# microsoft/ptgnn

Measured on AMD Instinct MI355X. Metric: edges/sec per MP layer, higher is better.
Workload: dtype f32; 1 GPU; cfg3: Graph2Class-style batch, 48 graphs N=115772, T0=8->T=17, E=625130 (incl. reverse+self), Typilus GGNN arch: 8 GGNN layers H=128 (+concat residual), max; hidden=128, mode=forward (inference), fp32, plan_build_in_step=True, message_rows=shared per (edge type, source) pair, parallelism=single GPU, minibatches_rotated=4

## Files before the change

ptgnn_amd/csrc/stream_gemm.hip:

```cpp
#include <stdlib.h>

#include "dense_common.h"
#include <atomic>

#include "stream_gemm.h"

namespace ptgnn_amd {
namespace {

using u32x4 = __attribute__((ext_vector_type(4))) uint32_t;

constexpr int kLdsBudget = 160 * 1024;
constexpr size_t kEpiBytes = 16 + 8 * 8 * 36 * sizeof(float);

__device__ __forceinline__ f32x16 zero16() {
  f32x16 v;
#pragma unroll
  for (int r = 0; r < 16; ++r) v[r] = 0.f;
  return v;
}

struct ARows {
  const float *c0, *c1, *n0, *n1;
};

__device__ __forceinline__ float4 load_piece(const ARows &r, int cc, int ch0, int nch, int g) {
  const bool nx = cc >= nch;
  const int c = nx ? cc - nch : cc;
  const float *b0 = nx ? r.n0 : r.c0;
  const float *b1 = nx ? r.n1 : r.c1;
  const float *p = c < ch0 ? b0 + c * 32 : b1 + (c - ch0) * 32;
  return *reinterpret_cast<const float4 *>(p + g * 8);
}

__device__ __forceinline__ int lane_piece_offset(int hi) { return hi * 4; }

template <int NBLK, int NACC, int PH, bool GRU>
__device__ __forceinline__ void chunk_f32(f32x16 (&acc)[NACC], float4 (&buf)[4], float4 (&bcur)[NBLK],
                                          const float *bl, int cbs, int kofs, int kofs_next, const ARows &rows,
                                          int cnext, int ch0, int nch) {
#pragma unroll
  for (int g = 0; g < 4; ++g) {
    float4 bn[NBLK];
    const int ko = g < 3 ? kofs + (g + 1) * 8 : kofs_next;
#pragma unroll
    for (int n = 0; n < NBLK; ++n) bn[n] = *reinterpret_cast<const float4 *>(bl + n * cbs + ko);
    __builtin_amdgcn_sched_barrier(0);
    const float4 a = buf[g];
#define PTGNN_STEP(C)                                                                     \
    _Pragma("unroll") for (int n = 0; n < NBLK; ++n) {                                    \
      const int t = (GRU && PH == 1 && n == 2) ? 3 : n;                                   \
      acc[t] = __builtin_amdgcn_mfma_f32_32x32x2f32(a.C, bcur[n].C, acc[t], 0, 0, 0);     \
    }
    PTGNN_STEP(x) PTGNN_STEP(y) PTGNN_STEP(z) PTGNN_STEP(w)
#undef PTGNN_STEP
    __builtin_amdgcn_sched_barrier(0);
#pragma unroll
    for (int n = 0; n < NBLK; ++n) bcur[n] = bn[n];
  }
#pragma unroll
  for (int g = 0; g < 4; ++g) {
    buf[g] = load_piece(rows, cnext, ch0, nch, g);
    __builtin_amdgcn_sched_barrier(0);
  }
}

struct Slab {
  int ld;
  __device__ __forceinline__ Slab(int K, int ) { ld = K + 4; }
  static size_t bytes(int K, int rows) { return (size_t)rows * (K + 4) * 4; }

  __device__ __forceinline__ void put4(float *smem, int r, int k, float4 v) const {
    *reinterpret_cast<float4 *>(smem + r * ld + k) = v;
  }
};

template <int NT, typename SrcFn, typename LiveFn>
__device__ __forceinline__ void fill_slab(float *smem, const Slab &sl, int rows, int kq, SrcFn src, LiveFn live) {
  constexpr int UB = 8;
  const int total = rows * kq;
  for (int i0 = threadIdx.x; i0 < total; i0 += NT * UB) {
    float4 v[UB];
    int rr[UB], qq[UB];
#pragma unroll
    for (int u = 0; u < UB; ++u) {
      const int i = i0 + u * NT;
      const int ic = i < total ? i : total - 1;
      rr[u] = ic / kq;
      qq[u] = ic - rr[u] * kq;
    }
#pragma unroll
    for (int u = 0; u < UB; ++u) {
      v[u] = *reinterpret_cast<const float4 *>(src(rr[u], qq[u]));
      __builtin_amdgcn_sched_barrier(0);
    }
#pragma unroll
    for (int u = 0; u < UB; ++u) {
      if (i0 + u * NT < total) sl.put4(smem, rr[u], qq[u] * 4, live(rr[u]) ? v[u] : make_float4(0.f, 0.f, 0.f, 0.f));
    }
  }
}

template <int NBLK, int NACC, bool GRU>
__device__ __forceinline__ void unit_kloop(f32x16 (&acc)[NACC], float4 (&a0)[4], float4 (&a1)[4],
                                           const float *smem, const Slab &sl, int li, int hi,
                                           const ARows &rows, int ch0, int nch) {
  const float *bl = smem + li * sl.ld + hi * 4;
  const int cbs = 32 * sl.ld;
  const int e0 = GRU ? ch0 : nch;
  float4 bcur[NBLK];
#pragma unroll
  for (int n = 0; n < NBLK; ++n) bcur[n] = *reinterpret_cast<const float4 *>(bl + n * cbs);
  for (int c = 0; c < e0; c += 2) {
    const int kn = c + 2 < nch ? c * 32 + 64 : 0;
    chunk_f32<NBLK, NACC, 0, GRU>(acc, a0, bcur, bl, cbs, c * 32, c * 32 + 32, rows, c + 2, ch0, nch);
    chunk_f32<NBLK, NACC, 0, GRU>(acc, a1, bcur, bl, cbs, c * 32 + 32, kn, rows, c + 3, ch0, nch);
  }
  if constexpr (GRU) {
    for (int c = ch0; c < nch; c += 2) {
      const int kn = c + 2 < nch ? c * 32 + 64 : 0;
      chunk_f32<NBLK, NACC, 1, GRU>(acc, a0, bcur, bl, cbs, c * 32, c * 32 + 32, rows, c + 2, ch0, nch);
      chunk_f32<NBLK, NACC, 1, GRU>(acc, a1, bcur, bl, cbs, c * 32 + 32, kn, rows, c + 3, ch0, nch);
    }
  }
}

__device__ __forceinline__ void prologue_loads(float4 (&a0)[4], float4 (&a1)[4], const ARows &rows, int ch0,
                                               int nch) {
#pragma unroll
  for (int g = 0; g < 4; ++g) {
    a0[g] = load_piece(rows, 0, ch0, nch, g);
    __builtin_amdgcn_sched_barrier(0);
  }
#pragma unroll
  for (int g = 0; g < 4; ++g) {
    a1[g] = load_piece(rows, 1, ch0, nch, g);
    __builtin_amdgcn_sched_barrier(0);
  }
}

__device__ __forceinline__ void unit_fence() {
  __builtin_amdgcn_s_waitcnt(0x0F70);
  __builtin_amdgcn_sched_barrier(0);
}

__device__ __forceinline__ int claim_unit(int *counter) {
  int v = 0;
  if ((threadIdx.x & 63) == 0) v = atomicAdd(counter, 1);
  return __builtin_amdgcn_readfirstlane(v);
}

constexpr int kTqLd = 36;
constexpr int kTqFloats = 8 * kTqLd;

__device__ __forceinline__ float4 tq_transpose(float *tq, int lane, int li, int hi, float v0, float v1, float v2,
                                               float v3) {
  float *w = tq + (4 * hi) * kTqLd + li;
  w[0] = v0; w[kTqLd] = v1; w[2 * kTqLd] = v2; w[3 * kTqLd] = v3;
  __builtin_amdgcn_wave_barrier();
  const float4 o = *reinterpret_cast<const float4 *>(tq + (lane >> 3) * kTqLd + (lane & 7) * 4);
  __builtin_amdgcn_wave_barrier();
  return o;
}

__device__ __forceinline__ void tq_untranspose(float *tq, int lane, int li, int hi, float4 in, float (&v)[4]) {
  *reinterpret_cast<float4 *>(tq + (lane >> 3) * kTqLd + (lane & 7) * 4) = in;
  __builtin_amdgcn_wave_barrier();
  const float *r = tq + (4 * hi) * kTqLd + li;
  v[0] = r[0]; v[1] = r[kTqLd]; v[2] = r[2 * kTqLd]; v[3] = r[3 * kTqLd];
  __builtin_amdgcn_wave_barrier();
}

using u32x4 = __attribute__((ext_vector_type(4))) uint32_t;

__device__ __forceinline__ __amdgpu_buffer_rsrc_t rows_descriptor(float *base , int64_t ld, int64_t rows_left,
                                                                  int width ) {
  const uint64_t b = reinterpret_cast<uint64_t>(base);
  const uint32_t lo = __builtin_amdgcn_readfirstlane((uint32_t)b), hi = __builtin_amdgcn_readfirstlane((uint32_t)(b >> 32));
  const int64_t rows = rows_left < 32 ? rows_left : 32;
  const int64_t bytes = rows > 0 ? ((rows - 1) * ld + width) * 4 : 0;
  return __builtin_amdgcn_make_buffer_rsrc(reinterpret_cast<float *>(((uint64_t)hi << 32) | lo), 0,
                                           __builtin_amdgcn_readfirstlane((int)bytes), 0x00020000);
}

__device__ __forceinline__ void store_row4(__amdgpu_buffer_rsrc_t rsrc, int lane_bytes, int uniform_bytes, float4 o) {
  const u32x4 v = {__float_as_uint(o.x), __float_as_uint(o.y), __float_as_uint(o.z), __float_as_uint(o.w)};
  __builtin_amdgcn_raw_buffer_store_b128(v, rsrc, lane_bytes + uniform_bytes, 0, 0);
}

template <int ACT, bool BIAS = true>
__device__ __forceinline__ void store_block_tq(const f32x16 &c, float *tq, float *yblk ,
                                               int64_t ld_y, float bv, int64_t rows_left, int lane, int li, int hi,
                                               const float *addblk = nullptr, int64_t ld_add = 0) {
  auto val = [&](int r) { return BIAS ? act_apply<ACT>(c[r] + bv) : act_apply<ACT>(c[r]); };
  float4 addv[4];
  if (addblk) {
#pragma unroll
    for (int q = 0; q < 4; ++q) {
      int64_t r = 8 * q + (lane >> 3);
      r = r < rows_left ? r : rows_left - 1;
      addv[q] = *reinterpret_cast<const float4 *>(addblk + r * ld_add + (lane & 7) * 4);
    }
  }
// ... 46 lines not shown

template <int NB>
__device__ __forceinline__ void linear_epilogue(const LinearArgs &p, f32x16 (&acc)[NB], float *tq, int64_t row0,
                                                int col_base, int lane, int li, int hi) {
#pragma unroll
  for (int n = 0; n < NB; ++n) {
    const int col = col_base + n * 32 + li;
    if (col_base + n * 32 < p.n_out) {
      const float bv = p.bias ? p.bias[col] : 0.f;
      if (p.vec_store) {
        float *yb = p.y + row0 * p.ld_y + col_base + n * 32;
        const int64_t left = p.rows - row0;
        if (p.bias) {
#pragma unroll
          for (int r = 0; r < 16; ++r) acc[n][r] += bv;
        }
        const float *ab = p.addend ? p.addend + row0 * p.ld_add + col_base + n * 32 : nullptr;
        if (p.act == PTGNN_AMD_ACT_TANH) store_block_tq<PTGNN_AMD_ACT_TANH, false>(acc[n], tq, yb, p.ld_y, 0.f, left, lane, li, hi, ab, p.ld_add);
        else if (p.act == PTGNN_AMD_ACT_RELU) store_block_tq<PTGNN_AMD_ACT_RELU, false>(acc[n], tq, yb, p.ld_y, 0.f, left, lane, li, hi, ab, p.ld_add);
        else store_block_tq<PTGNN_AMD_ACT_NONE, false>(acc[n], tq, yb, p.ld_y, 0.f, left, lane, li, hi, ab, p.ld_add);
      } else {
        float *yp = p.y + (row0 + 4 * hi) * p.ld_y + col;
        if (p.act == PTGNN_AMD_ACT_TANH) store_block<PTGNN_AMD_ACT_TANH>(acc[n], yp, p.ld_y, bv, row0, p.rows, hi);
        else if (p.act == PTGNN_AMD_ACT_RELU) store_block<PTGNN_AMD_ACT_RELU>(acc[n], yp, p.ld_y, bv, row0, p.rows, hi);
        else store_block<PTGNN_AMD_ACT_NONE>(acc[n], yp, p.ld_y, bv, row0, p.rows, hi);
      }
    }
    acc[n] = zero16();
  }
}

template <int NB>
__global__ __launch_bounds__(512, 2) void k_stream_linear(LinearArgs p) {
  extern __shared__ __attribute__((aligned(16))) float smem[];
  constexpr int NT = 512, BN = 32 * NB;
  const int b = blockIdx.x, G = gridDim.x;
  int slab, part;
  if (G % (kNumXcd * p.ncs) == 0) {
    const int xcd = b % kNumXcd, j = b / kNumXcd;
    slab = j % p.ncs;
    part = xcd + kNumXcd * (j / p.ncs);
  } else {
    slab = b / p.rps;
    part = b % p.rps;
  }
  const int rb0 = part * p.run_len;
  const int rb1 = rb0 + p.run_len < p.nrb ? rb0 + p.run_len : p.nrb;
  if (rb0 >= rb1) return;
  const int count = rb1 - rb0;

  const Slab sl(p.K, BN);
  int *counter = reinterpret_cast<int *>(smem + p.lds_floats);
  float *const tq = smem + p.lds_floats + 4 + (threadIdx.x >> 6) * kTqFloats;
  if (threadIdx.x == 0) *counter = 0;
  const int col_base = slab * BN;
  fill_slab<NT>(smem, sl, BN, p.K >> 2,
                       [&](int r, int q) {
                         const int wr = col_base + r < p.n_out ? col_base + r : p.n_out - 1;
                         return p.w + (int64_t)wr * p.K + q * 4;
                       },
                       [&](int r) { return col_base + r < p.n_out; });
  __syncthreads();

  const int lane = threadIdx.x & 63;
  const int li = lane & 31, hi = lane >> 5;
  const int nch = p.K >> 5;
  const int lofs = lane_piece_offset(hi);
  auto rowp = [&](int u) {
    int64_t row = (int64_t)(rb0 + (u < count ? u : count - 1)) * 32 + li;
    row = row < p.rows ? row : p.rows - 1;
    return p.x + row * p.ld_x + lofs;
  };
  int cur = claim_unit(counter);
  if (cur >= count) return;
  int nxt = claim_unit(counter);
  ARows rows;
  rows.c0 = rows.c1 = rowp(cur);
  rows.n0 = rows.n1 = rowp(nxt);
  float4 a0[4], a1[4];
  prologue_loads(a0, a1, rows, nch, nch);
  f32x16 acc[NB];
#pragma unroll
  for (int n = 0; n < NB; ++n) acc[n] = zero16();

  while (cur < count) {
    const int nn = claim_unit(counter);
    unit_fence();
    unit_kloop<NB, NB, false>(acc, a0, a1, smem, sl, li, hi, rows, nch, nch);
    const int64_t row0 = (int64_t)(rb0 + cur) * 32;
    linear_epilogue<NB>(p, acc, tq, row0, col_base, lane, li, hi);
    cur = nxt;
    nxt = nn;
    rows.c0 = rows.c1 = rows.n0;
    rows.n0 = rows.n1 = rowp(nxt);
  }
}

struct GruArgs {
  const float *a; int64_t ld_a; const float *h; int64_t ld_h;
  const float *w_ih, *w_hh, *b_ih, *b_hh;
  int64_t n; int M, H;
  float *out; int64_t ld_out; float *gates;
  int nrb, ncs, rps, run_len;
  int lds_floats;
};

__device__ __forceinline__ float fast_sigmoid(float v) {
  return __builtin_amdgcn_rcpf(1.0f + __builtin_amdgcn_exp2f(-1.4426950408889634f * v));
}

using f32x2 = __attribute__((ext_vector_type(2))) float;
__device__ __forceinline__ f32x2 splat2(float v) { return f32x2{v, v}; }
__device__ __forceinline__ f32x2 rcp_1_plus_exp2(f32x2 t) {
  const f32x2 d = f32x2{__builtin_amdgcn_exp2f(t.x), __builtin_amdgcn_exp2f(t.y)} + splat2(1.0f);
  return f32x2{__builtin_amdgcn_rcpf(d.x), __builtin_amdgcn_rcpf(d.y)};
}

__device__ __forceinline__ void gru_epilogue(const GruArgs &p, const f32x16 (&acc)[4], float *tq, int64_t row0,
                                             int j0, int lane, int li, int hi, float bir, float biz, float bin,
                                             float bhr, float bhz, float bhn) {
  const int trow = lane >> 3, tcol = (lane & 7) * 4;
#ifndef PTGNN_GLOBAL_STORES
  const __amdgpu_buffer_rsrc_t out_rsrc = rows_descriptor(p.out + row0 * p.ld_out + j0, p.ld_out, p.n - row0, 32);
  const __amdgpu_buffer_rsrc_t gate_rsrc =
      rows_descriptor(p.gates ? p.gates + row0 * (int64_t)(4 * p.H) + j0 : p.out, 4 * (int64_t)p.H, p.n - row0, 3 * p.H + 32);
#endif
#pragma unroll
  for (int q = 0; q < 4; ++q) {
    int64_t hrow = row0 + 8 * q + trow;
    const bool rvalid = hrow < p.n;
    hrow = rvalid ? hrow : p.n - 1;
    float hp[4];
    tq_untranspose(tq, lane, li, hi, *reinterpret_cast<const float4 *>(p.h + hrow * p.ld_h + j0 + tcol), hp);
// ... 18 lines not shown
    }
    const float4 o = tq_transpose(tq, lane, li, hi, res[0], res[1], res[2], res[3]);
#ifdef PTGNN_GLOBAL_STORES
    if (rvalid) *reinterpret_cast<float4 *>(p.out + hrow * p.ld_out + j0 + tcol) = o;
#else
    store_row4(out_rsrc, trow * (int)p.ld_out * 4 + tcol * 4, 8 * q * (int)p.ld_out * 4, o);
#endif
    if (p.gates) {
      const float4 o_r = tq_transpose(tq, lane, li, hi, rg[0], rg[1], rg[2], rg[3]);
      const float4 o_z = tq_transpose(tq, lane, li, hi, zg[0], zg[1], zg[2], zg[3]);
      const float4 o_n = tq_transpose(tq, lane, li, hi, ng[0], ng[1], ng[2], ng[3]);
      const float4 o_h = tq_transpose(tq, lane, li, hi, hn[0], hn[1], hn[2], hn[3]);
#ifdef PTGNN_GLOBAL_STORES
      float *gp = p.gates + hrow * (int64_t)(4 * p.H) + j0 + tcol;
      if (rvalid) {
        *reinterpret_cast<float4 *>(gp) = o_r;
        *reinterpret_cast<float4 *>(gp + p.H) = o_z;
        *reinterpret_cast<float4 *>(gp + 2 * p.H) = o_n;
        *reinterpret_cast<float4 *>(gp + 3 * p.H) = o_h;
      }
#else
      const int gl = trow * 16 * p.H + tcol * 4, gu = 8 * q * 16 * p.H;
      store_row4(gate_rsrc, gl, gu, o_r);
      store_row4(gate_rsrc, gl, gu + 4 * p.H, o_z);
      store_row4(gate_rsrc, gl, gu + 8 * p.H, o_n);
      store_row4(gate_rsrc, gl, gu + 12 * p.H, o_h);
#endif
    }
  }
}

__global__ __launch_bounds__(512, 2) void k_stream_gru(GruArgs p) {
  extern __shared__ __attribute__((aligned(16))) float smem[];
  constexpr int NT = 512;
  const int b = blockIdx.x, G = gridDim.x;
  int slab, part;
  if (G % (kNumXcd * p.ncs) == 0) {
    const int xcd = b % kNumXcd, j = b / kNumXcd;
    slab = j % p.ncs;
    part = xcd + kNumXcd * (j / p.ncs);
  } else {
    slab = b / p.rps;
    part = b % p.rps;
  }
  const int rb0 = part * p.run_len;
  const int rb1 = rb0 + p.run_len < p.nrb ? rb0 + p.run_len : p.nrb;
  if (rb0 >= rb1) return;
  const int count = rb1 - rb0;

  const int K = p.M + p.H;
  const Slab sl(K, 96);
  int *counter = reinterpret_cast<int *>(smem + p.lds_floats);
  float *const tq = smem + p.lds_floats + 4 + (threadIdx.x >> 6) * kTqFloats;
  if (threadIdx.x == 0) *counter = 0;
  const int j0 = slab * 32;
  {
    const int mq = p.M >> 2;
    fill_slab<NT>(smem, sl, 96, K >> 2,
                         [&](int r, int q) {
                           const int gate = r >> 5, jj = j0 + (r & 31);
                           return q < mq ? p.w_ih + ((int64_t)gate * p.H + jj) * p.M + q * 4
                                         : p.w_hh + ((int64_t)gate * p.H + jj) * p.H + (q - mq) * 4;
                         },
                         [](int) { return true; });
  }
  __syncthreads();

  const int lane = threadIdx.x & 63;
  const int li = lane & 31, hi = lane >> 5;
  const int ch0 = p.M >> 5, nch = K >> 5;
  const int lofs = lane_piece_offset(hi);
  auto clampr = [&](int u) {
    const int64_t row = (int64_t)(rb0 + (u < count ? u : count - 1)) * 32 + li;
    return row < p.n ? row : p.n - 1;
  };
  int cur = claim_unit(counter);
  if (cur >= count) return;
  int nxt = claim_unit(counter);
  ARows rows;
  {
    const int64_t r0 = clampr(cur), r1 = clampr(nxt);
    rows.c0 = p.a + r0 * p.ld_a + lofs; rows.c1 = p.h + r0 * p.ld_h + lofs;
    rows.n0 = p.a + r1 * p.ld_a + lofs; rows.n1 = p.h + r1 * p.ld_h + lofs;
  }
  float4 a0[4], a1[4];
  prologue_loads(a0, a1, rows, ch0, nch);
  f32x16 acc[4];
#pragma unroll
  for (int n = 0; n < 4; ++n) acc[n] = zero16();

  const int j = j0 + li;
  const float bir = p.b_ih[j], biz = p.b_ih[p.H + j], bin = p.b_ih[2 * p.H + j];
  const float bhr = p.b_hh[j], bhz = p.b_hh[p.H + j], bhn = p.b_hh[2 * p.H + j];

  while (cur < count) {
    const int nn = claim_unit(counter);
    unit_fence();
    unit_kloop<3, 4, true>(acc, a0, a1, smem, sl, li, hi, rows, ch0, nch);
    gru_epilogue(p, acc, tq, (int64_t)(rb0 + cur) * 32, j0, lane, li, hi, bir, biz, bin, bhr, bhz, bhn);
#pragma unroll
    for (int n = 0; n < 4; ++n) acc[n] = zero16();
    cur = nxt;
    nxt = nn;
    rows.c0 = rows.n0; rows.c1 = rows.n1;
    const int64_t r1 = clampr(nxt);
    rows.n0 = p.a + r1 * p.ld_a + lofs; rows.n1 = p.h + r1 * p.ld_h + lofs;
  }
}

constexpr int kRingPanel = 64;
constexpr int kRingLd = kRingPanel + 4;
constexpr int kRingPanelFloats = 96 * kRingLd;
constexpr int kRingWaves = 4;

__global__ __launch_bounds__(kRingWaves * 64, 2) void k_stream_gru_ring(GruArgs p) {
  extern __shared__ __attribute__((aligned(16))) float smem[];
  const int b = blockIdx.x, G = gridDim.x;
  int slab, part;
  if (G % (kNumXcd * p.ncs) == 0) {
    const int xcd = b % kNumXcd, j = b / kNumXcd;
    slab = j % p.ncs;
    part = xcd + kNumXcd * (j / p.ncs);
  } else {
    slab = b / p.rps;
    part = b % p.rps;
  }
  const int rb0 = part * p.run_len;
  const int rb1 = rb0 + p.run_len < p.nrb ? rb0 + p.run_len : p.nrb;
  if (rb0 >= rb1) return;
  const int count = rb1 - rb0;
  const int rounds = (count + kRingWaves - 1) / kRingWaves;

  const int K = p.M + p.H;
  const int npan = K / kRingPanel;
  const int lane = threadIdx.x & 63, wave = threadIdx.x >> 6;
  const int li = lane & 31, hi = lane >> 5;
  float *const tq = smem + 2 * kRingPanelFloats + wave * kTqFloats;
  const int j0 = slab * 32;
  const int ch0 = p.M >> 5, nch = K >> 5;
// ... 150 lines not shown
      for (int n = 0; n < 4; ++n) bcur[n] = *reinterpret_cast<const float4 *>(bl + n * cbs);
      chunk_f32<4, 4, 0, false>(acc, a0, bcur, bl, cbs, 0, 32, rows, 2 * pan + 2, nch, nch);
      *reinterpret_cast<float4 *>(nb) = w0;
      *reinterpret_cast<float4 *>(nb + 16 * kRingLd) = w1;
      *reinterpret_cast<float4 *>(nb + 32 * kRingLd) = w2;
      *reinterpret_cast<float4 *>(nb + 48 * kRingLd) = w3;
      w0 = *reinterpret_cast<const float4 *>(src + 4 * wq);
      w1 = *reinterpret_cast<const float4 *>(src + 5 * wq);
      w2 = *reinterpret_cast<const float4 *>(src + 6 * wq);
      w3 = *reinterpret_cast<const float4 *>(src + 7 * wq);
      __builtin_amdgcn_sched_barrier(0);
      chunk_f32<4, 4, 0, false>(acc, a1, bcur, bl, cbs, 32, 0, rows, 2 * pan + 3, nch, nch);
      *reinterpret_cast<float4 *>(nb + 64 * kRingLd) = w0;
      *reinterpret_cast<float4 *>(nb + 80 * kRingLd) = w1;
      *reinterpret_cast<float4 *>(nb + 96 * kRingLd) = w2;
      *reinterpret_cast<float4 *>(nb + 112 * kRingLd) = w3;
      lds_barrier();
    }
    if (u < count) linear_epilogue<4>(p, acc, tq, (int64_t)(rb0 + u) * 32, col_base, lane, li, hi);
#pragma unroll
    for (int n = 0; n < 4; ++n) acc[n] = zero16();
    rows.c0 = rows.c1 = rows.n0;
    rows.n0 = rows.n1 = rowp(u + 2 * kRingWaves);
  }
}

struct TablePrefixes {
  int v_wg, v_unit, wg_total, unit_total;
  __device__ __forceinline__ explicit TablePrefixes(const StreamEdgeTable &tab) {
    const int l = threadIdx.x & 63;
    v_wg = tab.wg_off[l];
    v_unit = tab.unit_off[l];
    wg_total = tab.wg_off[kStreamMaxTypes];
    unit_total = tab.unit_off[kStreamMaxTypes];
  }
  __device__ __forceinline__ static int entry(int v, int total, int i) {
    return i >= kStreamMaxTypes ? total : __builtin_amdgcn_readlane(v, i);
  }
  __device__ __forceinline__ void run_of_workgroup(int wg, int &u, int &u_end) const {
    const int lo = __popcll(__ballot(v_wg <= wg)) - 1;
    const int wg0 = entry(v_wg, wg_total, lo), u0 = entry(v_unit, unit_total, lo);
    const int64_t w = entry(v_wg, wg_total, lo + 1) - wg0, part = wg - wg0;
    const int64_t units = entry(v_unit, unit_total, lo + 1) - u0;
    u = u0 + (int)(part * units / w);
    u_end = u0 + (int)((part + 1) * units / w);
  }
  __device__ __forceinline__ void type_of_unit(int u, int &t, int &u0, int &u1) const {
    t = __popcll(__ballot(v_unit <= u)) - 1;
    u0 = entry(v_unit, unit_total, t);
    u1 = entry(v_unit, unit_total, t + 1);
  }
};

struct EdgeArgs {
  StreamEdgeTable tab;
  const StreamEdgeTable *tab_dev;
  const float *x; int64_t ld_x; int H; int use_dst; int M; int act;
  float *msg; int64_t ld_msg; int64_t msg_row_base;
  int64_t num_rows;
  int run_len, lds_floats;
};

#ifndef PTGNN_EDGE_WAVES
#define PTGNN_EDGE_WAVES 8
#endif
constexpr int kEdgeWaves = PTGNN_EDGE_WAVES;

template <int NB, bool INDIRECT>
__global__ __launch_bounds__(kEdgeWaves * 64, kEdgeWaves == 8 ? 2 : 3) void k_stream_edge(EdgeArgs p) {
  extern __shared__ __attribute__((aligned(16))) float smem[];
  constexpr int NT = kEdgeWaves * 64, BN = 32 * NB;
  const StreamEdgeTable *tabp;
  if constexpr (INDIRECT) tabp = p.tab_dev; else tabp = &p.tab;
  const StreamEdgeTable &tab = *tabp;
  const TablePrefixes tp(tab);
  if constexpr (INDIRECT) {
    if ((int)blockIdx.x >= tp.wg_total) return;
  }
  int u, u_end;
  tp.run_of_workgroup((int)blockIdx.x, u, u_end);
  if (u >= u_end) return;
  const int K = p.use_dst ? 2 * p.H : p.H;
  const Slab sl(K, BN);
  int *counter = reinterpret_cast<int *>(smem + p.lds_floats);
  float *const tq = smem + p.lds_floats + 4 + (threadIdx.x >> 6) * kTqFloats;
  const int lane = threadIdx.x & 63;
  const int li = lane & 31, hi = lane >> 5;
  const int ch0 = p.H >> 5, nch = K >> 5;
  const int lofs = lane_piece_offset(hi);

  while (u < u_end) {
    int t, t_u0, t_u1;
    tp.type_of_unit(u, t, t_u0, t_u1);
    const int seg_end = t_u1 < u_end ? t_u1 : u_end;
    const int ub = u - t_u0;
    const int count = seg_end - u;
    const int64_t type_row0 = tab.edge_off[t];
    const int64_t n_edges = tab.edge_off[t + 1] - type_row0;
    using GlobalIds = const __attribute__((address_space(1))) int64_t *;
    const GlobalIds src = (GlobalIds)tab.src[t];
    const GlobalIds dst = (GlobalIds)tab.dst[t];
    __syncthreads();
    if (threadIdx.x == 0) *counter = 0;
    {
      const float *w = p.tab.w[t];
      fill_slab<NT>(smem, sl, BN, K >> 2,
                           [&](int r, int q) { return w + (int64_t)(r < p.M ? r : p.M - 1) * K + q * 4; },
                           [&](int r) { return r < p.M; });
    }
    __syncthreads();

    int cur = claim_unit(counter);
    if (cur < count) {
      int nxt = claim_unit(counter);
      int nn = claim_unit(counter);
          auto edge_of = [&](int unit) {
        const int64_t e = (int64_t)(ub + (unit < count ? unit : count - 1)) * 32 + li;
        return e < n_edges ? e : n_edges - 1;
      };
      auto node_row = [&](int64_t id) {
        id = id < 0 ? 0 : id;
        return p.x + (id < p.num_rows ? id : p.num_rows - 1) * p.ld_x + lofs;
      };
      ARows rows;
      {
        const int64_t e0 = edge_of(cur), e1 = edge_of(nxt);
        rows.c0 = node_row(src[e0]); rows.c1 = node_row(dst[e0]);
        rows.n0 = node_row(src[e1]); rows.n1 = node_row(dst[e1]);
      }
      float4 a0[4], a1[4];
      prologue_loads(a0, a1, rows, ch0, nch);
      f32x16 acc[NB];
#pragma unroll
      for (int n = 0; n < NB; ++n) acc[n] = zero16();
      while (cur < count) {
        const int n3 = claim_unit(counter);
        const int64_t e_nn = edge_of(nn);
        unit_fence();
        const int64_t s_nn = src[e_nn], d_nn = dst[e_nn];
        unit_kloop<NB, NB, false>(acc, a0, a1, smem, sl, li, hi, rows, ch0, nch);
        const int64_t e_row0 = (int64_t)(ub + cur) * 32;
        const int64_t out_row0 = p.msg_row_base + type_row0 + e_row0;
#pragma unroll
        for (int n = 0; n < NB; ++n) {
          if (n * 32 < p.M) {
            float *yb = p.msg + out_row0 * p.ld_msg + n * 32;
            const int64_t left = n_edges - e_row0;
            if (p.act == PTGNN_AMD_ACT_TANH) store_block_tq<PTGNN_AMD_ACT_TANH, false>(acc[n], tq, yb, p.ld_msg, 0.f, left, lane, li, hi);
            else if (p.act == PTGNN_AMD_ACT_RELU) store_block_tq<PTGNN_AMD_ACT_RELU, false>(acc[n], tq, yb, p.ld_msg, 0.f, left, lane, li, hi);
            else store_block_tq<PTGNN_AMD_ACT_NONE, false>(acc[n], tq, yb, p.ld_msg, 0.f, left, lane, li, hi);
          }
          acc[n] = zero16();
        }
        cur = nxt; nxt = nn; nn = n3;
        rows.c0 = rows.n0; rows.c1 = rows.n1;
        rows.n0 = node_row(s_nn); rows.n1 = node_row(d_nn);
      }
    }
    u = seg_end;
  }
}

}

__device__ float4 ptgnn_amd_edge_store_sink[64 + 32];

namespace {

struct EdgeV2Args {
  EdgeArgs e;
  const uint32_t *mask;
  int mask_ld;
  int mask_col0;
  float scale;
};

__device__ __forceinline__ float keep_scaled(float v, uint32_t m, int bit, float scale) {
  const int t = ((int)(m << (31 - bit))) >> 31;
  return __uint_as_float(__float_as_uint(v * scale) & (uint32_t)t);
}

template <int NB, int DROP>
__device__ __forceinline__ void chunk_v2(f32x16 (&acc)[NB], float4 (&buf)[4], uint32_t &mw, float4 (&bcur)[NB],
                                         const float *bl, int cbs, int kofs, int kofs_next, const float *refill,
                                         const uint32_t *mrefill, int hi, float scale) {
  uint32_t m = 0;
  if constexpr (DROP == 1) m = mw >> (4 * hi);
#pragma unroll
  for (int g = 0; g < 4; ++g) {
    float4 bn[NB];
    const int ko = g < 3 ? kofs + (g + 1) * 8 : kofs_next;
#pragma unroll
    for (int n = 0; n < NB; ++n) bn[n] = *reinterpret_cast<const float4 *>(bl + n * cbs + ko);
    __builtin_amdgcn_sched_barrier(0);
    float4 a = buf[g];
    if constexpr (DROP == 1) {
      a.x = keep_scaled(a.x, m, 8 * g + 0, scale); a.y = keep_scaled(a.y, m, 8 * g + 1, scale);
      a.z = keep_scaled(a.z, m, 8 * g + 2, scale); a.w = keep_scaled(a.w, m, 8 * g + 3, scale);
    }
#define PTGNN_STEP(C)                                                                     \
    _Pragma("unroll") for (int n = 0; n < NB; ++n)                                        \
      acc[n] = __builtin_amdgcn_mfma_f32_32x32x2f32(a.C, bcur[n].C, acc[n], 0, 0, 0);
    PTGNN_STEP(x) PTGNN_STEP(y) PTGNN_STEP(z) PTGNN_STEP(w)
#undef PTGNN_STEP
    __builtin_amdgcn_sched_barrier(0);
#pragma unroll
    for (int n = 0; n < NB; ++n) bcur[n] = bn[n];
  }
  if constexpr (DROP == 1) {
    mw = *mrefill;
    __builtin_amdgcn_sched_barrier(0);
  }
#pragma unroll
  for (int g = 0; g < 4; ++g) {
    buf[g] = *reinterpret_cast<const float4 *>(refill + g * 8);
    __builtin_amdgcn_sched_barrier(0);
  }
}

template <int NB, int NCH, int DROP, int VAR>
__global__ __launch_bounds__(512, 2) void k_stream_edge_v2(EdgeV2Args q) {
  constexpr bool INDIRECT = VAR == 1;
  constexpr int CH0 = VAR == 2 ? NCH / 2 : NCH;
  extern __shared__ __attribute__((aligned(16))) float smem[];
  constexpr int NT = 512, BN = 32 * NB, K = 32 * NCH;
  const EdgeArgs &p = q.e;
  const StreamEdgeTable *tabp;
  if constexpr (INDIRECT) tabp = p.tab_dev; else tabp = &p.tab;
  const StreamEdgeTable &tab = *tabp;
  const TablePrefixes tp(tab);
  if constexpr (INDIRECT) {
    if ((int)blockIdx.x >= tp.wg_total) return;
  }
  int u, u_end;
  tp.run_of_workgroup((int)blockIdx.x, u, u_end);
  if (u >= u_end) return;
  const Slab sl(K, BN);
  int *counter = reinterpret_cast<int *>(smem + p.lds_floats);
  float *const tq = smem + p.lds_floats + 4 + (threadIdx.x >> 6) * kTqFloats;
  const int lane = threadIdx.x & 63;
  const int li = lane & 31, hi = lane >> 5;
  const int lofs = hi * 4;
  const int srow = lane >> 3, scol = (lane & 7) * 4;
  [[maybe_unused]] float *const sink = reinterpret_cast<float *>(ptgnn_amd_edge_store_sink) + lane * 4;
  const float *const bl = smem + li * sl.ld + hi * 4;
  const int cbs = 32 * sl.ld;

  while (u < u_end) {
    int t, t_u0, t_u1;
    tp.type_of_unit(u, t, t_u0, t_u1);
    const int seg_end = t_u1 < u_end ? t_u1 : u_end;
    const int ub = u - t_u0;
    const int count = seg_end - u;
    const int64_t type_row0 = tab.edge_off[t];
    const int64_t n_edges = tab.edge_off[t + 1] - type_row0;
    using GlobalIds = const __attribute__((address_space(1))) int64_t *;
    const GlobalIds src = (GlobalIds)tab.src[t];
    const GlobalIds dst = (GlobalIds)tab.dst[t];
    __syncthreads();
    if (threadIdx.x == 0) *counter = 0;
    {
      const float *w = p.tab.w[t];
      fill_slab<NT>(smem, sl, BN, K >> 2, [&](int r, int q) { return w + (int64_t)r * K + q * 4; },
                           [](int) { return true; });
    }
    __syncthreads();

    int cur = claim_unit(counter);
    if (cur < count) {
      int nxt = claim_unit(counter);
      auto edge_of = [&](int unit) {
        const int64_t e = (int64_t)(ub + (unit < count ? unit : count - 1)) * 32 + li;
        return e < n_edges ? e : n_edges - 1;
      };
      auto node_row = [&](int64_t id) {
        id = id < 0 ? 0 : id;
        return p.x + (id < p.num_rows ? id : p.num_rows - 1) * p.ld_x + lofs;
      };
      auto chunk_ptr = [&](const float *r0, const float *r1, int cc) {
        return cc < CH0 ? r0 + cc * 32 : r1 + (cc - CH0) * 32;
      };
      const int64_t mrow_base = p.msg_row_base + type_row0;
      auto mask_row = [&](int64_t e) { return q.mask + (mrow_base + e) * q.mask_ld; };

      const float *c0, *c1, *n0, *n1;
      const uint32_t *mc = nullptr, *mn = nullptr;
      {
        const int64_t e0 = edge_of(cur);
        c0 = node_row(src[e0]); c1 = node_row(dst[e0]);
        if constexpr (DROP == 1) mc = mask_row(e0);
      }
      float4 a0[4], a1[4];
      uint32_t m0 = 0, m1 = 0;
      if constexpr (DROP == 1) { m0 = mc[0]; __builtin_amdgcn_sched_barrier(0); }
#pragma unroll
      for (int g = 0; g < 4; ++g) {
        a0[g] = *reinterpret_cast<const float4 *>(chunk_ptr(c0, c1, 0) + g * 8);
        __builtin_amdgcn_sched_barrier(0);
      }
      if constexpr (DROP == 1) { m1 = mc[1]; __builtin_amdgcn_sched_barrier(0); }
#pragma unroll
      for (int g = 0; g < 4; ++g) {
        a1[g] = *reinterpret_cast<const float4 *>(chunk_ptr(c0, c1, 1) + g * 8);
        __builtin_amdgcn_sched_barrier(0);
      }
      int64_t e_n = edge_of(nxt);
      int64_t s_n = src[e_n], d_n = dst[e_n];
      __builtin_amdgcn_sched_barrier(0);
      f32x16 acc[NB];
#pragma unroll
      for (int n = 0; n < NB; ++n) acc[n] = zero16();
      float4 bcur[NB];
#pragma unroll
      for (int n = 0; n < NB; ++n) bcur[n] = *reinterpret_cast<const float4 *>(bl + n * cbs);

      while (true) {
// ... 410 lines not shown
```

Measured before the change: 1.296 billion edges/s.

## Overlap weight-slab fill with first A-row loads and deepen fill batching

In the linear, GRU and edge streaming kernels, each wave now takes its first units statically (wave, wave+NW) instead of claiming them atomically. It issues the first gathered row loads before the LDS weight slab is filled, so global latency for activations overlaps with the weight fill. The fill is restructured into larger load batches (up to 24 float4 per thread) with incremental index math. The edge kernel also keeps edge-type table entries in lanes and reads them with readlane, avoiding scalar memory trips per segment. This adds register pressure from the deeper batches and changes unit assignment, which could hurt occupancy or load balance.

```diff
diff --git a/ptgnn_amd/csrc/stream_gemm.hip b/ptgnn_amd/csrc/stream_gemm.hip
--- a/ptgnn_amd/csrc/stream_gemm.hip
+++ b/ptgnn_amd/csrc/stream_gemm.hip
@@ -75,8 +75,36 @@
   }
 };
 
+#ifndef PTGNN_FILL_MAX_BATCH
+#define PTGNN_FILL_MAX_BATCH 24
+#endif
+
+template <int NT, int UB, typename SrcFn, typename LiveFn>
+__device__ __forceinline__ void fill_batch(float *smem, const Slab &sl, int rows, int kq, int total, int i0, SrcFn src,
+                                           LiveFn live) {
+  float4 v[UB];
+  int dst[UB];
+  const int dr = NT / kq, dq = NT - dr * kq;
+  int r = i0 / kq, q = i0 - r * kq;
+#pragma unroll
+  for (int u = 0; u < UB; ++u) {
+    const bool in = i0 + u * NT < total;
+    const int rr = in ? r : rows - 1, qq = in ? q : kq - 1;
+    dst[u] = in ? (((rr * sl.ld + qq * 4) << 1) | (live(rr) ? 1 : 0)) : -1;
+    v[u] = *reinterpret_cast<const float4 *>(src(rr, qq));
+    __builtin_amdgcn_sched_barrier(0);
+    r += dr; q += dq;
+    if (q >= kq) { q -= kq; ++r; }
+  }
+#pragma unroll
+  for (int u = 0; u < UB; ++u) {
+    if (dst[u] >= 0)
+      *reinterpret_cast<float4 *>(smem + (dst[u] >> 1)) = (dst[u] & 1) ? v[u] : make_float4(0.f, 0.f, 0.f, 0.f);
+  }
+}
+
 template <int NT, typename SrcFn, typename LiveFn>
-__device__ __forceinline__ void fill_slab(float *smem, const Slab &sl, int rows, int kq, SrcFn src, LiveFn live) {
+__device__ __forceinline__ void fill_slab_depth8(float *smem, const Slab &sl, int rows, int kq, SrcFn src, LiveFn live) {
   constexpr int UB = 8;
   const int total = rows * kq;
   for (int i0 = threadIdx.x; i0 < total; i0 += NT * UB) {
@@ -99,6 +127,23 @@
       if (i0 + u * NT < total) sl.put4(smem, rr[u], qq[u] * 4, live(rr[u]) ? v[u] : make_float4(0.f, 0.f, 0.f, 0.f));
     }
   }
+}
+
+template <int NT, int MAXB, typename SrcFn, typename LiveFn>
+__device__ __forceinline__ void fill_slab(float *smem, const Slab &sl, int rows, int kq, SrcFn src, LiveFn live) {
+  constexpr int kMax = MAXB < PTGNN_FILL_MAX_BATCH ? MAXB : PTGNN_FILL_MAX_BATCH;
+  const int total = rows * kq;
+  int base = 0;
+  if constexpr (kMax >= 24) {
+    for (; total - base > 16 * NT; base += 24 * NT) fill_batch<NT, 24>(smem, sl, rows, kq, total, base + (int)threadIdx.x, src, live);
+  }
+  if constexpr (kMax >= 16) {
+    if (total - base > 8 * NT) {
+      fill_batch<NT, 16>(smem, sl, rows, kq, total, base + (int)threadIdx.x, src, live);
+      base += 16 * NT;
+    }
+  }
+  for (; base < total; base += 8 * NT) fill_batch<NT, 8>(smem, sl, rows, kq, total, base + (int)threadIdx.x, src, live);
 }
 
 template <int NBLK, int NACC, bool GRU>
@@ -149,6 +194,7 @@
   if ((threadIdx.x & 63) == 0) v = atomicAdd(counter, 1);
   return __builtin_amdgcn_readfirstlane(v);
 }
+
 
 constexpr int kTqLd = 36;
 constexpr int kTqFloats = 8 * kTqLd;
@@ -301,17 +347,11 @@
   const Slab sl(p.K, BN);
   int *counter = reinterpret_cast<int *>(smem + p.lds_floats);
   float *const tq = smem + p.lds_floats + 4 + (threadIdx.x >> 6) * kTqFloats;
-  if (threadIdx.x == 0) *counter = 0;
+  constexpr int NW = NT / 64;
+  if (threadIdx.x == 0) *counter = 2 * NW;
   const int col_base = slab * BN;
-  fill_slab<NT>(smem, sl, BN, p.K >> 2,
-                       [&](int r, int q) {
-                         const int wr = col_base + r < p.n_out ? col_base + r : p.n_out - 1;
-                         return p.w + (int64_t)wr * p.K + q * 4;
-                       },
-                       [&](int r) { return col_base + r < p.n_out; });
-  __syncthreads();
-
-  const int lane = threadIdx.x & 63;
+
+  const int lane = threadIdx.x & 63, wave = threadIdx.x >> 6;
   const int li = lane & 31, hi = lane >> 5;
   const int nch = p.K >> 5;
   const int lofs = lane_piece_offset(hi);
@@ -320,14 +360,20 @@
     row = row < p.rows ? row : p.rows - 1;
     return p.x + row * p.ld_x + lofs;
   };
-  int cur = claim_unit(counter);
-  if (cur >= count) return;
-  int nxt = claim_unit(counter);
+  int cur = wave, nxt = wave + NW;
   ARows rows;
   rows.c0 = rows.c1 = rowp(cur);
   rows.n0 = rows.n1 = rowp(nxt);
   float4 a0[4], a1[4];
   prologue_loads(a0, a1, rows, nch, nch);
+  fill_slab<NT, 24>(smem, sl, BN, p.K >> 2,
+                       [&](int r, int q) {
+                         const int wr = col_base + r < p.n_out ? col_base + r : p.n_out - 1;
+                         return p.w + (int64_t)wr * p.K + q * 4;
+                       },
+                       [&](int r) { return col_base + r < p.n_out; });
+  __syncthreads();
+  if (cur >= count) return;
   f32x16 acc[NB];
 #pragma unroll
   for (int n = 0; n < NB; ++n) acc[n] = zero16();
@@ -452,21 +498,11 @@
   const Slab sl(K, 96);
   int *counter = reinterpret_cast<int *>(smem + p.lds_floats);
   float *const tq = smem + p.lds_floats + 4 + (threadIdx.x >> 6) * kTqFloats;
-  if (threadIdx.x == 0) *counter = 0;
+  constexpr int NW = NT / 64;
+  if (threadIdx.x == 0) *counter = 2 * NW;
   const int j0 = slab * 32;
-  {
-    const int mq = p.M >> 2;
-    fill_slab<NT>(smem, sl, 96, K >> 2,
-                         [&](int r, int q) {
-                           const int gate = r >> 5, jj = j0 + (r & 31);
-                           return q < mq ? p.w_ih + ((int64_t)gate * p.H + jj) * p.M + q * 4
-                                         : p.w_hh + ((int64_t)gate * p.H + jj) * p.H + (q - mq) * 4;
-                         },
-                         [](int) { return true; });
-  }
-  __syncthreads();
-
-  const int lane = threadIdx.x & 63;
+
+  const int lane = threadIdx.x & 63, wave = threadIdx.x >> 6;
   const int li = lane & 31, hi = lane >> 5;
   const int ch0 = p.M >> 5, nch = K >> 5;
   const int lofs = lane_piece_offset(hi);
@@ -474,9 +510,7 @@
     const int64_t row = (int64_t)(rb0 + (u < count ? u : count - 1)) * 32 + li;
     return row < p.n ? row : p.n - 1;
   };
-  int cur = claim_unit(counter);
-  if (cur >= count) return;
-  int nxt = claim_unit(counter);
+  int cur = wave, nxt = wave + NW;
   ARows rows;
   {
     const int64_t r0 = clampr(cur), r1 = clampr(nxt);
@@ -485,6 +519,18 @@
   }
   float4 a0[4], a1[4];
   prologue_loads(a0, a1, rows, ch0, nch);
+  {
+    const int mq = p.M >> 2;
+    fill_slab<NT, 24>(smem, sl, 96, K >> 2,
+                         [&](int r, int q) {
+                           const int gate = r >> 5, jj = j0 + (r & 31);
+                           return q < mq ? p.w_ih + ((int64_t)gate * p.H + jj) * p.M + q * 4
+                                         : p.w_hh + ((int64_t)gate * p.H + jj) * p.H + (q - mq) * 4;
+                         },
+                         [](int) { return true; });
+  }
+  __syncthreads();
+  if (cur >= count) return;
   f32x16 acc[4];
 #pragma unroll
   for (int n = 0; n < 4; ++n) acc[n] = zero16();
@@ -741,6 +787,26 @@
   }
 };
 
+struct TableEntries {
+  int64_t v_off, off_total;
+  const int64_t *v_src, *v_dst;
+  __device__ __forceinline__ explicit TableEntries(const StreamEdgeTable &tab) {
+    const int l = threadIdx.x & 63;
+    v_off = tab.edge_off[l];
+    off_total = tab.edge_off[kStreamMaxTypes];
+    v_src = tab.src[l];
+    v_dst = tab.dst[l];
+  }
+  __device__ __forceinline__ static int64_t lane64(int64_t v, int i) {
+    const uint32_t lo = (uint32_t)__builtin_amdgcn_readlane((int)(uint32_t)v, i);
+    const uint32_t hi = (uint32_t)__builtin_amdgcn_readlane((int)(uint32_t)((uint64_t)v >> 32), i);
+    return (int64_t)(((uint64_t)hi << 32) | lo);
+  }
+  __device__ __forceinline__ int64_t edge_off(int i) const { return i >= kStreamMaxTypes ? off_total : lane64(v_off, i); }
+  __device__ __forceinline__ uint64_t src_of(int t) const { return (uint64_t)lane64((int64_t)reinterpret_cast<uint64_t>(v_src), t); }
+  __device__ __forceinline__ uint64_t dst_of(int t) const { return (uint64_t)lane64((int64_t)reinterpret_cast<uint64_t>(v_dst), t); }
+};
+
 struct EdgeArgs {
   StreamEdgeTable tab;
   const StreamEdgeTable *tab_dev;
@@ -763,6 +829,9 @@
   if constexpr (INDIRECT) tabp = p.tab_dev; else tabp = &p.tab;
   const StreamEdgeTable &tab = *tabp;
   const TablePrefixes tp(tab);
+#ifndef PTGNN_TABLE_TWO_TRIPS
+  const TableEntries te(tab);
+#endif
   if constexpr (INDIRECT) {
     if ((int)blockIdx.x >= tp.wg_total) return;
   }
@@ -773,10 +842,175 @@
   const Slab sl(K, BN);
   int *counter = reinterpret_cast<int *>(smem + p.lds_floats);
   float *const tq = smem + p.lds_floats + 4 + (threadIdx.x >> 6) * kTqFloats;
-  const int lane = threadIdx.x & 63;
+  const int lane = threadIdx.x & 63, wave = threadIdx.x >> 6;
   const int li = lane & 31, hi = lane >> 5;
   const int ch0 = p.H >> 5, nch = K >> 5;
   const int lofs = lane_piece_offset(hi);
+  constexpr int NW = kEdgeWaves;
+
+  for (int seg = 0; u < u_end; ++seg) {
+    int t, t_u0, t_u1;
+    tp.type_of_unit(u, t, t_u0, t_u1);
+    const int seg_end = t_u1 < u_end ? t_u1 : u_end;
+    const int ub = u - t_u0;
+    const int count = seg_end - u;
+    using GlobalIds = const __attribute__((address_space(1))) int64_t *;
+#ifndef PTGNN_TABLE_TWO_TRIPS
+    const int64_t type_row0 = te.edge_off(t);
+    const int64_t n_edges = te.edge_off(t + 1) - type_row0;
+    const GlobalIds src = (GlobalIds)te.src_of(t);
+    const GlobalIds dst = (GlobalIds)te.dst_of(t);
+#else
+    const int64_t type_row0 = tab.edge_off[t];
+    const int64_t n_edges = tab.edge_off[t + 1] - type_row0;
+    const GlobalIds src = (GlobalIds)tab.src[t];
+    const GlobalIds dst = (GlobalIds)tab.dst[t];
+#endif
+    auto edge_of = [&](int unit) {
+      const int64_t e = (int64_t)(ub + (unit < count ? unit : count - 1)) * 32 + li;
+      return e < n_edges ? e : n_edges - 1;
+    };
+    auto node_row = [&](int64_t id) {
+      id = id < 0 ? 0 : id;
+      return p.x + (id < p.num_rows ? id : p.num_rows - 1) * p.ld_x + lofs;
+    };
+    int cur = wave, nxt = wave + NW, nn = wave + 2 * NW;
+    ARows rows;
+    {
+      const int64_t e0 = edge_of(cur), e1 = edge_of(nxt);
+      const int64_t s0 = src[e0], d0 = dst[e0], s1 = src[e1], d1 = dst[e1];
+      __builtin_amdgcn_sched_barrier(0);
+      rows.c0 = node_row(s0); rows.c1 = node_row(d0);
+      rows.n0 = node_row(s1); rows.n1 = node_row(d1);
+    }
+    float4 a0[4], a1[4];
+    prologue_loads(a0, a1, rows, ch0, nch);
+    if (seg > 0) __syncthreads();
+    if (threadIdx.x == 0) *counter = 3 * NW;
+    {
+      const float *w = p.tab.w[t];
+      fill_slab<NT, 16>(smem, sl, BN, K >> 2,
+                           [&](int r, int q) { return w + (int64_t)(r < p.M ? r : p.M - 1) * K + q * 4; },
+                           [&](int r) { return r < p.M; });
+    }
+    __syncthreads();
+
+    if (cur < count) {
+      f32x16 acc[NB];
+#pragma unroll
+      for (int n = 0; n < NB; ++n) acc[n] = zero16();
+      while (cur < count) {
+        const int n3 = claim_unit(counter);
+        const int64_t e_nn = edge_of(nn);
+        unit_fence();
+        const int64_t s_nn = src[e_nn], d_nn = dst[e_nn];
+        unit_kloop<NB, NB, false>(acc, a0, a1, smem, sl, li, hi, rows, ch0, nch);
+        const int64_t e_row0 = (int64_t)(ub + cur) * 32;
+        const int64_t out_row0 = p.msg_row_base + type_row0 + e_row0;
+#pragma unroll
+        for (int n = 0; n < NB; ++n) {
+          if (n * 32 < p.M) {
+            float *yb = p.msg + out_row0 * p.ld_msg + n * 32;
+            const int64_t left = n_edges - e_row0;
+            if (p.act == PTGNN_AMD_ACT_TANH) store_block_tq<PTGNN_AMD_ACT_TANH, false>(acc[n], tq, yb, p.ld_msg, 0.f, left, lane, li, hi);
+            else if (p.act == PTGNN_AMD_ACT_RELU) store_block_tq<PTGNN_AMD_ACT_RELU, false>(acc[n], tq, yb, p.ld_msg, 0.f, left, lane, li, hi);
+            else store_block_tq<PTGNN_AMD_ACT_NONE, false>(acc[n], tq, yb, p.ld_msg, 0.f, left, lane, li, hi);
+          }
+          acc[n] = zero16();
+        }
+        cur = nxt; nxt = nn; nn = n3;
+        rows.c0 = rows.n0; rows.c1 = rows.n1;
+        rows.n0 = node_row(s_nn); rows.n1 = node_row(d_nn);
+      }
+    }
+    u = seg_end;
+  }
+}
+
+}
+
+__device__ float4 ptgnn_amd_edge_store_sink[64 + 32];
+
+namespace {
+
+struct EdgeV2Args {
+  EdgeArgs e;
+  const uint32_t *mask;
+  int mask_ld;
+  int mask_col0;
+  float scale;
+};
+
+__device__ __forceinline__ float keep_scaled(float v, uint32_t m, int bit, float scale) {
+  const int t = ((int)(m << (31 - bit))) >> 31;
+  return __uint_as_float(__float_as_uint(v * scale) & (uint32_t)t);
+}
+
+template <int NB, int DROP>
+__device__ __forceinline__ void chunk_v2(f32x16 (&acc)[NB], float4 (&buf)[4], uint32_t &mw, float4 (&bcur)[NB],
+                                         const float *bl, int cbs, int kofs, int kofs_next, const float *refill,
+                                         const uint32_t *mrefill, int hi, float scale) {
+  uint32_t m = 0;
+  if constexpr (DROP == 1) m = mw >> (4 * hi);
+#pragma unroll
+  for (int g = 0; g < 4; ++g) {
+    float4 bn[NB];
+    const int ko = g < 3 ? kofs + (g + 1) * 8 : kofs_next;
+#pragma unroll
+    for (int n = 0; n < NB; ++n) bn[n] = *reinterpret_cast<const float4 *>(bl + n * cbs + ko);
+    __builtin_amdgcn_sched_barrier(0);
+    float4 a = buf[g];
+    if constexpr (DROP == 1) {
+      a.x = keep_scaled(a.x, m, 8 * g + 0, scale); a.y = keep_scaled(a.y, m, 8 * g + 1, scale);
+      a.z = keep_scaled(a.z, m, 8 * g + 2, scale); a.w = keep_scaled(a.w, m, 8 * g + 3, scale);
+    }
+#define PTGNN_STEP(C)                                                                     \
+    _Pragma("unroll") for (int n = 0; n < NB; ++n)                                        \
+      acc[n] = __builtin_amdgcn_mfma_f32_32x32x2f32(a.C, bcur[n].C, acc[n], 0, 0, 0);
+    PTGNN_STEP(x) PTGNN_STEP(y) PTGNN_STEP(z) PTGNN_STEP(w)
+#undef PTGNN_STEP
+    __builtin_amdgcn_sched_barrier(0);
+#pragma unroll
+    for (int n = 0; n < NB; ++n) bcur[n] = bn[n];
+  }
+  if constexpr (DROP == 1) {
+    mw = *mrefill;
+    __builtin_amdgcn_sched_barrier(0);
+  }
+#pragma unroll
+  for (int g = 0; g < 4; ++g) {
+    buf[g] = *reinterpret_cast<const float4 *>(refill + g * 8);
+    __builtin_amdgcn_sched_barrier(0);
+  }
+}
+
+template <int NB, int NCH, int DROP, int VAR>
+__global__ __launch_bounds__(512, 2) void k_stream_edge_v2(EdgeV2Args q) {
+  constexpr bool INDIRECT = VAR == 1;
+  constexpr int CH0 = VAR == 2 ? NCH / 2 : NCH;
+  extern __shared__ __attribute__((aligned(16))) float smem[];
+  constexpr int NT = 512, BN = 32 * NB, K = 32 * NCH;
+  const EdgeArgs &p = q.e;
+  const StreamEdgeTable *tabp;
+  if constexpr (INDIRECT) tabp = p.tab_dev; else tabp = &p.tab;
+  const StreamEdgeTable &tab = *tabp;
+  const TablePrefixes tp(tab);
+  if constexpr (INDIRECT) {
+    if ((int)blockIdx.x >= tp.wg_total) return;
+  }
+  int u, u_end;
+  tp.run_of_workgroup((int)blockIdx.x, u, u_end);
+  if (u >= u_end) return;
+  const Slab sl(K, BN);
+  int *counter = reinterpret_cast<int *>(smem + p.lds_floats);
+  float *const tq = smem + p.lds_floats + 4 + (threadIdx.x >> 6) * kTqFloats;
+  const int lane = threadIdx.x & 63;
+  const int li = lane & 31, hi = lane >> 5;
+  const int lofs = hi * 4;
+  const int srow = lane >> 3, scol = (lane & 7) * 4;
+  [[maybe_unused]] float *const sink = reinterpret_cast<float *>(ptgnn_amd_edge_store_sink) + lane * 4;
+  const float *const bl = smem + li * sl.ld + hi * 4;
+  const int cbs = 32 * sl.ld;
 
   while (u < u_end) {
     int t, t_u0, t_u1;
@@ -793,164 +1027,7 @@
     if (threadIdx.x == 0) *counter = 0;
     {
       const float *w = p.tab.w[t];
-      fill_slab<NT>(smem, sl, BN, K >> 2,
-                           [&](int r, int q) { return w + (int64_t)(r < p.M ? r : p.M - 1) * K + q * 4; },
-                           [&](int r) { return r < p.M; });
-    }
-    __syncthreads();
-
-    int cur = claim_unit(counter);
-    if (cur < count) {
-      int nxt = claim_unit(counter);
-      int nn = claim_unit(counter);
-          auto edge_of = [&](int unit) {
-        const int64_t e = (int64_t)(ub + (unit < count ? unit : count - 1)) * 32 + li;
-        return e < n_edges ? e : n_edges - 1;
-      };
-      auto node_row = [&](int64_t id) {
-        id = id < 0 ? 0 : id;
-        return p.x + (id < p.num_rows ? id : p.num_rows - 1) * p.ld_x + lofs;
-      };
-      ARows rows;
-      {
-        const int64_t e0 = edge_of(cur), e1 = edge_of(nxt);
-        rows.c0 = node_row(src[e0]); rows.c1 = node_row(dst[e0]);
-        rows.n0 = node_row(src[e1]); rows.n1 = node_row(dst[e1]);
-      }
-      float4 a0[4], a1[4];
-      prologue_loads(a0, a1, rows, ch0, nch);
-      f32x16 acc[NB];
-#pragma unroll
-      for (int n = 0; n < NB; ++n) acc[n] = zero16();
-      while (cur < count) {
-        const int n3 = claim_unit(counter);
-        const int64_t e_nn = edge_of(nn);
-        unit_fence();
-        const int64_t s_nn = src[e_nn], d_nn = dst[e_nn];
-        unit_kloop<NB, NB, false>(acc, a0, a1, smem, sl, li, hi, rows, ch0, nch);
-        const int64_t e_row0 = (int64_t)(ub + cur) * 32;
-        const int64_t out_row0 = p.msg_row_base + type_row0 + e_row0;
-#pragma unroll
-        for (int n = 0; n < NB; ++n) {
-          if (n * 32 < p.M) {
-            float *yb = p.msg + out_row0 * p.ld_msg + n * 32;
-            const int64_t left = n_edges - e_row0;
-            if (p.act == PTGNN_AMD_ACT_TANH) store_block_tq<PTGNN_AMD_ACT_TANH, false>(acc[n], tq, yb, p.ld_msg, 0.f, left, lane, li, hi);
-            else if (p.act == PTGNN_AMD_ACT_RELU) store_block_tq<PTGNN_AMD_ACT_RELU, false>(acc[n], tq, yb, p.ld_msg, 0.f, left, lane, li, hi);
-            else store_block_tq<PTGNN_AMD_ACT_NONE, false>(acc[n], tq, yb, p.ld_msg, 0.f, left, lane, li, hi);
-          }
-          acc[n] = zero16();
-        }
-        cur = nxt; nxt = nn; nn = n3;
-        rows.c0 = rows.n0; rows.c1 = rows.n1;
-        rows.n0 = node_row(s_nn); rows.n1 = node_row(d_nn);
-      }
-    }
-    u = seg_end;
-  }
-}
-
-}
-
-__device__ float4 ptgnn_amd_edge_store_sink[64 + 32];
-
-namespace {
-
-struct EdgeV2Args {
-  EdgeArgs e;
-  const uint32_t *mask;
-  int mask_ld;
-  int mask_col0;
-  float scale;
-};
-
-__device__ __forceinline__ float keep_scaled(float v, uint32_t m, int bit, float scale) {
-  const int t = ((int)(m << (31 - bit))) >> 31;
-  return __uint_as_float(__float_as_uint(v * scale) & (uint32_t)t);
-}
-
-template <int NB, int DROP>
-__device__ __forceinline__ void chunk_v2(f32x16 (&acc)[NB], float4 (&buf)[4], uint32_t &mw, float4 (&bcur)[NB],
-                                         const float *bl, int cbs, int kofs, int kofs_next, const float *refill,
-                                         const uint32_t *mrefill, int hi, float scale) {
-  uint32_t m = 0;
-  if constexpr (DROP == 1) m = mw >> (4 * hi);
-#pragma unroll
-  for (int g = 0; g < 4; ++g) {
-    float4 bn[NB];
-    const int ko = g < 3 ? kofs + (g + 1) * 8 : kofs_next;
-#pragma unroll
-    for (int n = 0; n < NB; ++n) bn[n] = *reinterpret_cast<const float4 *>(bl + n * cbs + ko);
-    __builtin_amdgcn_sched_barrier(0);
-    float4 a = buf[g];
-    if constexpr (DROP == 1) {
-      a.x = keep_scaled(a.x, m, 8 * g + 0, scale); a.y = keep_scaled(a.y, m, 8 * g + 1, scale);
-      a.z = keep_scaled(a.z, m, 8 * g + 2, scale); a.w = keep_scaled(a.w, m, 8 * g + 3, scale);
-    }
-#define PTGNN_STEP(C)                                                                     \
-    _Pragma("unroll") for (int n = 0; n < NB; ++n)                                        \
-      acc[n] = __builtin_amdgcn_mfma_f32_32x32x2f32(a.C, bcur[n].C, acc[n], 0, 0, 0);
-    PTGNN_STEP(x) PTGNN_STEP(y) PTGNN_STEP(z) PTGNN_STEP(w)
-#undef PTGNN_STEP
-    __builtin_amdgcn_sched_barrier(0);
-#pragma unroll
-    for (int n = 0; n < NB; ++n) bcur[n] = bn[n];
-  }
-  if constexpr (DROP == 1) {
-    mw = *mrefill;
-    __builtin_amdgcn_sched_barrier(0);
-  }
-#pragma unroll
-  for (int g = 0; g < 4; ++g) {
-    buf[g] = *reinterpret_cast<const float4 *>(refill + g * 8);
-    __builtin_amdgcn_sched_barrier(0);
-  }
-}
-
-template <int NB, int NCH, int DROP, int VAR>
-__global__ __launch_bounds__(512, 2) void k_stream_edge_v2(EdgeV2Args q) {
-  constexpr bool INDIRECT = VAR == 1;
-  constexpr int CH0 = VAR == 2 ? NCH / 2 : NCH;
-  extern __shared__ __attribute__((aligned(16))) float smem[];
-  constexpr int NT = 512, BN = 32 * NB, K = 32 * NCH;
-  const EdgeArgs &p = q.e;
-  const StreamEdgeTable *tabp;
-  if constexpr (INDIRECT) tabp = p.tab_dev; else tabp = &p.tab;
-  const StreamEdgeTable &tab = *tabp;
-  const TablePrefixes tp(tab);
-  if constexpr (INDIRECT) {
-    if ((int)blockIdx.x >= tp.wg_total) return;
-  }
-  int u, u_end;
-  tp.run_of_workgroup((int)blockIdx.x, u, u_end);
-  if (u >= u_end) return;
-  const Slab sl(K, BN);
-  int *counter = reinterpret_cast<int *>(smem + p.lds_floats);
-  float *const tq = smem + p.lds_floats + 4 + (threadIdx.x >> 6) * kTqFloats;
-  const int lane = threadIdx.x & 63;
-  const int li = lane & 31, hi = lane >> 5;
-  const int lofs = hi * 4;
-  const int srow = lane >> 3, scol = (lane & 7) * 4;
-  [[maybe_unused]] float *const sink = reinterpret_cast<float *>(ptgnn_amd_edge_store_sink) + lane * 4;
-  const float *const bl = smem + li * sl.ld + hi * 4;
-  const int cbs = 32 * sl.ld;
-
-  while (u < u_end) {
-    int t, t_u0, t_u1;
-    tp.type_of_unit(u, t, t_u0, t_u1);
-    const int seg_end = t_u1 < u_end ? t_u1 : u_end;
-    const int ub = u - t_u0;
-    const int count = seg_end - u;
-    const int64_t type_row0 = tab.edge_off[t];
-    const int64_t n_edges = tab.edge_off[t + 1] - type_row0;
-    using GlobalIds = const __attribute__((address_space(1))) int64_t *;
-    const GlobalIds src = (GlobalIds)tab.src[t];
-    const GlobalIds dst = (GlobalIds)tab.dst[t];
-    __syncthreads();
-    if (threadIdx.x == 0) *counter = 0;
-    {
-      const float *w = p.tab.w[t];
-      fill_slab<NT>(smem, sl, BN, K >> 2, [&](int r, int q) { return w + (int64_t)r * K + q * 4; },
+      fill_slab_depth8<NT>(smem, sl, BN, K >> 2, [&](int r, int q) { return w + (int64_t)r * K + q * 4; },
                            [](int) { return true; });
     }
     __syncthreads();
```

Result: no change. 1.288 billion edges/s (-0.6%).
